# monahand1023/imageclust

Measured on AMD Instinct MI355X. Metric: images/sec (embed+Ward), higher is better.
Workload: dtype bf16; 1 GPU; the metric's size (configs[2]'s N=100000) on 1 GPU: 100000 synthetic 224x224x3 images (structured, seed 20250217; 100000 on this rank), ResNet50-v1 bf16 batch=256 -> 2048-d pooled E -> Ward min=5 max=50 (merge loop on GPU0) -> cluster ids on host; n_images_total=100000, embed_dim=2048, weights=synthetic seed 1, device=AMD Radeon Graphics (gfx950:sramecc+:xnack-)

## Files before the change

imageclust_amd/_lib.py:

```python
import ctypes as C
import os

import numpy as np

_HERE = os.path.dirname(os.path.abspath(__file__))
SO_PATH = os.environ.get("ICL_SO_PATH") or os.path.join(_HERE, "libimageclust_hip.so")

ICL_OK = 0
ICL_ERR_ARG, ICL_ERR_CONSTRAINT, ICL_ERR_HIP, ICL_ERR_NOMODEL, ICL_ERR_IO, ICL_ERR_UNSUPPORTED, ICL_ERR_OVERSIZE, ICL_ERR_NOMEM = range(1, 9)
HEAD_POOLED, HEAD_DENSE0 = 2048, 1000
PREC_FP32, PREC_BF16, PREC_BF16X3 = 0, 1, 2
UPDATE_EXACT, UPDATE_LW = 0, 1
SYNTH_NOISE, SYNTH_STRUCTURED = 0, 1
TILES_AUTO, TILES_LOCAL, TILES_DISTRIBUTED = 0, 1, 2
MERGE_GPU0, MERGE_SHARDED = 0, 1
CONV_P8_OFF, CONV_P8_AUTO, CONV_P8_ALL = 0, 1, 2
CONV_SPLIT = 16
ROWS_SINGLE, ROWS_EXACT_BATCH, ROWS_LW_BOUND, ROWS_LW_FAST = 0, 1, 2, 3
FILE_FAIL_NEXT_LEADER = 0x100
MANY_MID_AUTO, MANY_MID_OFF, MANY_MID_ON = 0, 1, 2
ENTROPY_HOST, ENTROPY_GPU = 0, 1
K_CONV, K_DIST_EXACT, K_DIST_MFMA, K_ROWMIN, K_UPDATE, K_EMBED_OTHER, K_CONV64 = range(7)
K_NAMES = ["conv_igemm_kernel<*,128>", "ward_dist_exact_kernel", "dist_mfma_kernel", "row_argmin_*_kernel",
           "ward_update_exact_kernel", "embed_other", "conv_igemm_kernel<*,64>"]
# ... 20 lines not shown
    ("icl_synthetic_blob_bytes", _i64, []),
    ("icl_synthetic_blob", _int, [C.c_uint64, _vp, _i64]),
    ("icl_embed_u8", _int, [_vp, _vp, _i64, _int, _int, _vp]),
    ("icl_embed_u8_dev", _int, [_vp, _vp, _i64, _int, _int, _vp]),
    ("icl_embed_file", _int, [_vp, C.c_char_p, _int, _vp]),
    ("icl_set_file_options", _int, [_vp, _int, _int, _int]),
    ("icl_file_batch_stats", _int, [_vp, _pi64, _pi64]),
    ("icl_preprocess_u8", _int, [_vp, _vp]),
    ("icl_preprocess_file", _int, [C.c_char_p, _vp]),
    ("icl_resize_u8", _int, [_vp, _i32, _i32, _vp, _i32, _i32]),
    ("icl_decode_image_file", _int, [C.c_char_p, _vp, _i64, _pi32, _pi32]),
    ("icl_load_image_224", _int, [C.c_char_p, _vp]),
    ("icl_load_images_224_dev", _int, [_vp, _vp, _i64, _i32, _vp, _vp]),
    ("icl_embed_files", _int, [_vp, _vp, _i64, _int, _int, _i32, _vp, _vp]),
    ("icl_embed_files_dev", _int, [_vp, _vp, _i64, _int, _int, _i32, _vp, _vp]),
    ("icl_last_ingest_stats", _int, [_vp, _pi64, _pi64, _pi64, _pd]),
    ("icl_set_ingest_options", _int, [_vp, _int]),
    ("icl_last_entropy_stats", _int, [_vp, _pi64, _pi64, _pi64, _pi64]),
    ("icl_jpeg_coefs_files", _int, [_vp, _vp, _i64, _int, _vp, _i64, _vp, _vp]),
    ("icl_jpeg_coefs_file_host", _int, [C.c_char_p, _int, _vp, _i64, _pi64, _vp]),
    ("icl_decode_image_mem", _int, [_vp, _i64, _vp, _i64, _pi32, _pi32]),
    ("icl_load_image_224_mem", _int, [_vp, _i64, _vp]),
    ("icl_preprocess_mem", _int, [_vp, _i64, _vp]),
    ("icl_embed_image_mem", _int, [_vp, _vp, _i64, _int, _vp]),
    ("icl_load_images_224_mem_dev", _int, [_vp, _vp, _vp, _i64, _i32, _vp, _vp]),
    ("icl_embed_images_mem", _int, [_vp, _vp, _vp, _i64, _int, _int, _i32, _vp, _vp]),
    ("icl_embed_images_mem_dev", _int, [_vp, _vp, _vp, _i64, _int, _int, _i32, _vp, _vp]),
    ("icl_cluster_requests_mem", _int, [_vp, _i32] + [_vp] * 8 + [_int, _int, _i32] + [_vp] * 8),
    ("icl_jpeg_coefs_mem", _int, [_vp, _vp, _vp, _i64, _int, _vp, _i64, _vp, _vp]),
    ("icl_set_batch", _int, [_vp, _int]),
    ("icl_set_conv_options", _int, [_vp, _int]),
    ("icl_conv_stats", _int, [_vp, _vp, _vp]),
    ("icl_conv_split_launches", _int, [_vp, _vp]),
    ("icl_conv2d_fused", _int, [_vp, _int, _vp, _int, _int, _int, _vp, _int, _int, _int, _int, _vp, _vp, _vp, _int, _vp]),
    ("icl_conv2d_dual", _int, [_vp, _int, _vp, _int, _int, _int, _vp, _vp, _int, _int, _vp, _int, _int, _vp, _vp, _int, _vp]),
    ("icl_embed_taps", _int, [_vp, _int, _vp, _int, _int, _vp]),
    ("icl_stem_pool", _int, [_vp, _int, _vp, _int, _vp]),
    ("icl_bottleneck56", _int, [_vp, _vp, _int, _int, _int, _int] + [_vp] * 13),
    ("icl_calc_optimal_clusters", _int, [_i64, _i64, _i64, _pi64]),
    ("icl_ward_distance_matrix", _int, [_vp, _vp, _vp, _i64, _i32, _vp, _i64]),
    ("icl_ward_distance_matrix_dev", _int, [_vp, _vp, _vp, _i64, _i32, _vp, _i64]),
    ("icl_merge_centroid", _int, [_vp, _vp, _i64, _vp, _i64, _i32, _vp]),
    ("icl_update_distance_matrix", _int, [_vp, _vp, _i64, _i64, _vp, _vp, _i32, _i64, _i64, _vp, _i64]),
    ("icl_find_closest", _int, [_vp, _vp, _i64, _i64, _pi64, _pi64]),
    ("icl_find_closest_dev", _int, [_vp, _vp, _i64, _i64, _pi64, _pi64]),
    ("icl_group_create", _int, [_pi32, _i32, C.POINTER(_vp)]),
    ("icl_group_destroy", None, [_vp]),
    ("icl_group_size", _i32, [_vp]),
    ("icl_group_ctx", _vp, [_vp, _i32]),
    ("icl_group_last_error", C.c_char_p, [_vp]),
    ("icl_group_load_onnx", _int, [_vp, C.c_char_p]),
    ("icl_group_load_blob", _int, [_vp, _vp, _i64]),
    ("icl_group_load_synthetic", _int, [_vp, C.c_uint64]),
    ("icl_group_embed_u8", _int, [_vp, _vp, _i64, _int, _int, _vp]),
    ("icl_group_cluster", _int, [_vp, _vp, _i64, _i32, _i32, _i32, _int, _vp, _vp, _pi32]),
    ("icl_set_ward_options", _int, [_vp, _int]),
    ("icl_embed_cluster_dev", _int, [_vp, _vp, _i64, _int, _i32, _i32, _int, _int, _vp, _vp, _vp, _pi32]),
    ("icl_group_embed_cluster", _int, [_vp, _vp, _i64, _int, _i32, _i32, _int, _vp, _vp, _vp, _pi32]),
    ("icl_ward_rows_partition", _int, [_i64, _i32, _i32, _pi64, _pi64]),
    ("icl_ward_span", _int, [_i64, _i64, _pi64, _pi64]),
    ("icl_ward_distance_rows_dev", _int, [_vp, _vp, _i64, _i32, _i64, _i64, _vp]),
    ("icl_ward_rows_hold_bounds", _int, [_vp, _i64, _int]),
    ("icl_ward_prepare", _int, [_vp, _i64, _i32]),
    ("icl_ward_unpack_spans_dev", _int, [_vp, _i32, _pi64, _pi64, C.POINTER(_vp)]),
    ("icl_group_set_options", _int, [_vp, _int, _int]),
    ("icl_cluster_prefilled_dev", _int, [_vp, _vp, _i64, _i32, _i32, _i32, _int, _i64, _i64, _vp, _vp, _pi32]),
# ... 249 lines not shown

        t = E if isinstance(E, torch.Tensor) else torch.from_numpy(np.ascontiguousarray(E, dtype=np.float32))
        t = t.to("cuda:%d" % self.device, dtype=torch.float32).contiguous()
        n, d = t.shape
        a, b, u = C.c_int64(0), C.c_int64(0), C.c_int64(0)
        g, v = C.c_double(0), C.c_double(0)
        check(self.h, self.L.icl_distance_bounds_check_dev(self.h, C.c_void_p(t.data_ptr()), n, d, kind, C.byref(a), C.byref(b), C.byref(u), C.byref(g), C.byref(v)))
        pairs = n * (n - 1) / 2
        return {"below": a.value, "above": b.value, "unflagged": u.value, "mean_gap": g.value / pairs, "mean_val": v.value / pairs}

    def load_synthetic(self, seed=1):
        check(self.h, self.L.icl_model_load_synthetic(self.h, seed))

    def load_blob(self, blob):
        buf = np.frombuffer(blob, np.uint8)
        check(self.h, self.L.icl_model_load_blob(self.h, buf.ctypes.data, buf.nbytes))

    def load_onnx(self, path):
        check(self.h, self.L.icl_model_load_onnx(self.h, os.fsencode(path)))

    def set_batch(self, b):
        check(self.h, self.L.icl_set_batch(self.h, b))

    def conv_stats(self):
        a, b = C.c_int64(0), C.c_int64(0)
        check(self.h, self.L.icl_conv_stats(self.h, C.byref(a), C.byref(b)))
        return a.value, b.value

    def conv_split_launches(self):
        a = C.c_int64(0)
        check(self.h, self.L.icl_conv_split_launches(self.h, C.byref(a)))
        return a.value

    def set_conv_options(self, p8_mode=1):
        check(self.h, self.L.icl_set_conv_options(self.h, p8_mode))

    def embed_u8(self, imgs, head=HEAD_POOLED, prec=PREC_FP32):
        imgs = np.ascontiguousarray(imgs, np.uint8).reshape(-1, IMG_BYTES)
        n = imgs.shape[0]
        out = np.empty((n, head), np.float32)
        check(self.h, self.L.icl_embed_u8(self.h, imgs.ctypes.data, n, head, prec, out.ctypes.data))
        return out

    def embed_u8_dev(self, d_imgs, n, d_out, head=HEAD_POOLED, prec=PREC_BF16):
        check(self.h, self.L.icl_embed_u8_dev(self.h, _vp(d_imgs), n, head, prec, _vp(d_out)))

    def embed_file(self, path, head=HEAD_DENSE0):
        out = np.empty(head, np.float32)
        check(self.h, self.L.icl_embed_file(self.h, os.fsencode(path), head, out.ctypes.data))
        return out

    def _files_call(self, fn, paths, *args):
        enc = [os.fsencode(p) for p in paths]
        arr = (C.c_char_p * max(1, len(enc)))(*enc)
        status = np.zeros(len(enc), np.int32)
        rc = fn(self.h, arr, len(enc), *args, status.ctypes.data)
        failed = np.flatnonzero(status)
        if rc != ICL_OK and not (failed.size and status[failed[0]] == rc):
            check(self.h, rc)
        return status

    def embed_image_mem(self, data, head=HEAD_DENSE0):
        p, n, keep = _byte_view(data)
        out = np.empty(head, np.float32)
        check(self.h, self.L.icl_embed_image_mem(self.h, _vp(p), n, head, out.ctypes.data))
        del keep
# ... 569 lines not shown
```

imageclust_amd/csrc/conv_wr.h:

```cpp
#pragma once
#include "mfma_tile.h"
#include "resnet_fused.h"

template <int NP>
__device__ __forceinline__ void wr_dma_chunk(const i32x4_t &srd, unsigned v0, unsigned v1, unsigned soff, unsigned lds0)
{
    unsigned keep;
    if constexpr (NP == 2)
        asm volatile("s_mov_b32 %0, m0\n\ts_mov_b32 m0, %5\n\ts_nop 4\n\tbuffer_load_dwordx4 %1, %3, %4 offen lds\n\t"
                     "s_mov_b32 m0, %6\n\ts_nop 0\n\tbuffer_load_dwordx4 %2, %3, %4 offen lds\n\ts_mov_b32 m0, %0"
                     : "=&s"(keep)
                     : "v"(v0), "v"(v1), "s"(srd), "s"(soff), "s"(lds0), "s"(lds0 + 4096u)
                     : "memory");
    else
        asm volatile("s_mov_b32 %0, m0\n\ts_mov_b32 m0, %4\n\ts_nop 4\n\tbuffer_load_dwordx4 %1, %2, %3 offen lds\n\ts_mov_b32 m0, %0"
                     : "=&s"(keep)
                     : "v"(v0), "s"(srd), "s"(soff), "s"(lds0)
                     : "memory");
}
template <int KC, int PT>
__device__ __forceinline__ void wr_dma(const i32x4_t &srd, unsigned v0, unsigned v1, unsigned lds0)
{
    static_assert(PT == 64 || PT == 32, "64- or 32-pixel tiles");
#pragma unroll
    for (int c = 0; c < KC; ++c) wr_dma_chunk<PT / 32>(srd, v0, v1, 128u * c, lds0 + (unsigned)(PT * 128) * c);
}

struct wr_args {
    const uint16_t *X;
    const uint16_t *W;
    const uint16_t *R;
    uint16_t *Y;
    const float *scale, *shift;
    int M, N, relu;
    int nslices, nworkers;
};

template <int K, int NS, int MT, bool RES>
__global__ __launch_bounds__(256, (K == 256 && MT == 2) ? 3 : 2) void conv_wr_kernel(const wr_args p)
{
    typedef unsigned u32x2_t __attribute__((ext_vector_type(2)));
    typedef unsigned u32x4_t __attribute__((ext_vector_type(4)));
    constexpr int KC = K / 64, KF = K / 32;
    constexpr int CW = NS / 4, NT = CW / 16;
    constexpr int PT = 16 * MT;
    constexpr int ABYTES = KC * PT * 128;
    static_assert(NT % 2 == 0 && NT * KF * 4 <= 128 && (MT == 4 || MT == 2), "pairs of accumulator tiles for the lane swap; <= 128 VGPRs of weights");
    __shared__ __attribute__((aligned(1024))) unsigned char smem[2 * ABYTES];
    const int tid = threadIdx.x, lane = tid & 63;
    const int wid = __builtin_amdgcn_readfirstlane(tid >> 6);
    const int l15 = lane & 15, q = lane >> 4;
    const int xcd = (int)blockIdx.x & 7, rr = (int)blockIdx.x >> 3;
    const int slice = rr % p.nslices, worker = (rr / p.nslices) * 8 + xcd;
    const int n0 = slice * NS + wid * CW;
    const int ntiles = (p.M + PT - 1) / PT;
    if (worker >= ntiles) return;

    u32x4_t wreg[NT][KF];
#pragma unroll
    for (int nt = 0; nt < NT; ++nt)
#pragma unroll
        for (int kf = 0; kf < KF; ++kf) wreg[nt][kf] = *reinterpret_cast<const u32x4_t *>(p.W + (size_t)(n0 + 16 * nt + l15) * K + 32 * kf + 8 * q);
    asm volatile("s_waitcnt vmcnt(0)" ::: "memory");
#pragma unroll
    for (int nt = 0; nt < NT; ++nt)
#pragma unroll
        for (int kf = 0; kf < KF; ++kf) asm volatile("" : "+v"(wreg[nt][kf]));
    const int cbl = (q & 1) * 16 + (q >> 1) * 8;
    float sc[NT / 2][8], sh[NT / 2][8];
#pragma unroll
    for (int i = 0; i < NT / 2; ++i) {
        const int c = n0 + i * 32 + cbl;
        const float4 a0 = *reinterpret_cast<const float4 *>(p.scale + c), a1 = *reinterpret_cast<const float4 *>(p.scale + c + 4);
        const float4 b0 = *reinterpret_cast<const float4 *>(p.shift + c), b1 = *reinterpret_cast<const float4 *>(p.shift + c + 4);
        sc[i][0] = a0.x; sc[i][1] = a0.y; sc[i][2] = a0.z; sc[i][3] = a0.w; sc[i][4] = a1.x; sc[i][5] = a1.y; sc[i][6] = a1.z; sc[i][7] = a1.w;
        sh[i][0] = b0.x; sh[i][1] = b0.y; sh[i][2] = b0.z; sh[i][3] = b0.w; sh[i][4] = b1.x; sh[i][5] = b1.y; sh[i][6] = b1.z; sh[i][7] = b1.w;
    }
    const i32x4_t xsrd = bn56_srd(p.X, (unsigned)((size_t)p.M * K * 2));
    const unsigned lds0 = __builtin_amdgcn_readfirstlane(lds_addr_of(smem) + wid * 1024);
    int drow[2];
    unsigned dsw[2];
#pragma unroll
    for (int j = 0; j < 2; ++j) {
        drow[j] = (j * 4 + wid) * 8 + (lane >> 3);
        dsw[j] = (unsigned)(((lane & 7) ^ ((drow[j] >> 1) & 7)) << 4);
    }
    auto stage = [&](int tile, int buf) {
        unsigned v[2];
#pragma unroll
        for (int j = 0; j < 2; ++j) {
            const int m = tile * PT + drow[j];
            v[j] = (tile < ntiles && m < p.M) ? (unsigned)m * (unsigned)(K * 2) + dsw[j] : BN56_OOB;
        }
        wr_dma<KC, PT>(xsrd, v[0], v[1], lds0 + buf * ABYTES);
    };
    const int fsw = (l15 >> 1) & 7;
    unsigned xoff[2];
#pragma unroll
    for (int s = 0; s < 2; ++s) xoff[s] = (unsigned)(l15 * 128 + ((((4 * s + q) ^ fsw) & 7) << 4));

    typedef uint16_t elem;
    const __amdgpu_buffer_rsrc_t rsrd = __builtin_amdgcn_make_buffer_rsrc((void *)(RES ? p.R : p.Y), 0, (int)((size_t)p.M * p.N * 2), 0x00020000);
    const __amdgpu_buffer_rsrc_t ysrd = __builtin_amdgcn_make_buffer_rsrc((void *)p.Y, 0, (int)((size_t)p.M * p.N * 2), 0x00020000);
    u32x4_t rv[MT][NT / 2];
    auto row_off = [&](int tile, int mt) -> unsigned {
        const int64_t m = (int64_t)tile * PT + mt * 16 + l15;
        return (tile < ntiles && m < p.M) ? (unsigned)((m * p.N + n0 + cbl) * 2) : BN56_OOB;
    };
    auto load_res = [&](int tile) {
        if (!RES) return;
#pragma unroll
        for (int mt = 0; mt < MT; ++mt) {
            const unsigned o = row_off(tile, mt);
#pragma unroll
            for (int i = 0; i < NT / 2; ++i) rv[mt][i] = __builtin_amdgcn_raw_buffer_load_b128(rsrd, (int)o, i * 64, 0);
        }
    };
    int tile = worker;
    stage(tile, 0);
    stage(tile + p.nworkers, 1);
    load_res(tile);
    asm volatile("s_waitcnt vmcnt(0)" ::: "memory");
    for (int it = 0; tile < ntiles; ++it, tile += p.nworkers) {
        const int buf = it & 1;
        __builtin_amdgcn_s_barrier();
        __builtin_amdgcn_sched_barrier(0);
        f32x4 acc[MT][NT];
// ... 26 lines not shown
        }
#pragma unroll
        for (int mt = 0; mt < MT; ++mt) {
            const unsigned o = row_off(tile, mt);
#pragma unroll
            for (int i = 0; i < NT / 2; ++i) {
                const f32x4 ta = acc[mt][2 * i], tb = acc[mt][2 * i + 1];
                float v[8];
#pragma unroll
                for (int j = 0; j < 4; ++j) {
                    const u32x2_t r = __builtin_amdgcn_permlane16_swap(__float_as_uint(ta[j]), __float_as_uint(tb[j]), false, false);
                    v[j] = __uint_as_float(r[0]);
                    v[4 + j] = __uint_as_float(r[1]);
                }
                const elem *re = reinterpret_cast<const elem *>(&rv[mt][i]);
                u32x4_t ov;
                elem *oe = reinterpret_cast<elem *>(&ov);
#pragma unroll
                for (int e = 0; e < 8; ++e) {
                    float y = v[e] * sc[i][e] + sh[i][e];
                    if (RES) y += BF16::to_f(re[e]);
                    if (p.relu) y = fmaxf(y, 0.0f);
                    oe[e] = BF16::from_f(y);
                }
                __builtin_amdgcn_raw_buffer_store_b128(ov, ysrd, (int)o, i * 64, 0);
            }
        }
        stage(tile + 2 * p.nworkers, buf);
        load_res(tile + p.nworkers);
    }
    asm volatile("s_waitcnt vmcnt(0)" ::: "memory");
}

static bool conv_wr_shape(const conv_args &a, int *ns, int *pt)
{
    static const int pt256 = [] {
        const char *e = getenv("ICL_WR_PT256");
        return e && atoi(e) == 32 ? 32 : 64;
    }();
    if (a.K == 128) { *ns = 256; *pt = 64; }
    else if (a.K == 256) { *ns = 128; *pt = pt256; }
    else if (a.K == 512) { *ns = 128; *pt = 32; }
    else return false;
    return a.Cout % *ns == 0;
}
static bool conv_wr_eligible(const conv_args &a, int mode)
{
    if (mode == 0 || a.X2 || a.KH != 1 || a.KW != 1 || a.stride != 1 || a.pad != 0 || a.Cin != a.K) return false;
    int ns, pt;
    if (!conv_wr_shape(a, &ns, &pt)) return false;
    if (a.K == 512 && a.Cout > 128 && a.Cout < 2048) return false;
    if ((size_t)a.M * a.K * 2 >= (1ull << 31) || (size_t)a.M * a.Cout * 2 >= (1ull << 31)) return false;
    return true;
}
template <int K, int NS, int MT>
static void launch_conv_wr_t(hipStream_t strm, const wr_args &w, dim3 grid, bool res)
{
    if (res) hipLaunchKernelGGL((conv_wr_kernel<K, NS, MT, true>), grid, dim3(256), 0, strm, w);
    else hipLaunchKernelGGL((conv_wr_kernel<K, NS, MT, false>), grid, dim3(256), 0, strm, w);
}
static void launch_conv_wr(icl_ctx *ctx, const conv_args &a)
{
    hipStream_t strm = ctx->cur_stream ? ctx->cur_stream : ctx->stream;
    wr_args w;
    w.X = (const uint16_t *)a.X; w.W = (const uint16_t *)a.Wt; w.R = (const uint16_t *)a.R; w.Y = (uint16_t *)a.Y;
    w.scale = a.scale; w.shift = a.shift; w.M = (int)a.M; w.N = a.Cout; w.relu = a.relu;
    int ns = 0, pt = 0;
    (void)conv_wr_shape(a, &ns, &pt);
    w.nslices = a.Cout / ns;
    const int ntiles = (int)icl_ceil_div(a.M, pt);
    const int per_cu = (a.K == 256 && pt == 32) ? 3 : 2;
    const int slots = per_cu * ctx->prop.multiProcessorCount;
    int nworkers = std::max(8, (slots / w.nslices) & ~7);
    nworkers = std::min(nworkers, (int)icl_ceil_div(ntiles, 8) * 8);
    w.nworkers = nworkers;
    const dim3 grid((unsigned)(w.nslices * nworkers));
    if (a.K == 128) launch_conv_wr_t<128, 256, 4>(strm, w, grid, a.R != nullptr);
    else if (a.K == 256 && pt == 64) launch_conv_wr_t<256, 128, 4>(strm, w, grid, a.R != nullptr);
    else if (a.K == 256) launch_conv_wr_t<256, 128, 2>(strm, w, grid, a.R != nullptr);
    else launch_conv_wr_t<512, 128, 2>(strm, w, grid, a.R != nullptr);
}
```

imageclust_amd/csrc/icl_common.h:

```cpp
#pragma once
#include <hip/hip_runtime.h>

#include <condition_variable>
#include <cstdarg>
#include <cstdint>
#include <cstdio>
#include <functional>
#include <mutex>
#include <string>
#include <vector>

#include "../../include/icl_model_format.h"
#include "../../include/imageclust.h"

#define ICL_MAXF 3.40282346638528859811704183484516925e+38f

struct icl_prof_slot {
    double ms = 0, flops = 0, bytes = 0;
    int64_t launches = 0;
};

struct icl_pending_event {
    hipEvent_t a, b;
    int kclass;
// ... 39 lines not shown
};

struct icl_sk_slot {
    hipStream_t stream = nullptr;
    void *part = nullptr;
    int *flag = nullptr;
    int cap = 0, epoch = 0;
};

struct icl_ward_report {
    std::vector<int32_t> merges;
    std::vector<float> merge_vals;
    int64_t bound_viol = 0;
    int32_t mode[2] = {0, 0};
    int64_t layout[3] = {0, 0, 0};
    int64_t stats[4] = {0, 0, 0, 0};
    double dist_ms = 0, merge_ms = 0;
};

struct icl_ctx {
    int device = 0;
    hipStream_t stream = nullptr;
    hipStream_t stream2 = nullptr;
    hipStream_t stream3 = nullptr;
    hipEvent_t ev_s3 = nullptr;
    std::function<int(int64_t, int64_t, hipEvent_t)> embed_hook;
    hipStream_t cur_stream = nullptr;
    hipEvent_t ev_fork = nullptr, ev_join = nullptr;
    std::mutex mu;
    std::string err;
    hipDeviceProp_t prop;
    int batch = 256;
    int64_t conv_launches[2] = {0, 0};
    int conv_wr = 1;
    int conv_sk = 0;
    int conv_sk_min_k = 2048;
    int64_t conv_sk_launches = 0;
    icl_sk_slot sk[8];
    int conv_p8 = 1;
    int ward_dist = 0;
    int prof_mask = 0;
    icl_prof_slot prof[ICL_K_NCLASS];
    std::vector<icl_pending_event> pending;
    std::vector<hipEvent_t> event_pool;
    double last_embed_ms = 0;
    icl_ward_report last;
    int64_t ward_wide_fail_n = 0;
    icl_model *model = nullptr;
    icl_ward_ws *ward = nullptr;
    icl_ward_shard *shard = nullptr;
    int shard_rank = 0;
    int64_t *ward_rowoff = nullptr;
    int64_t ward_rowoff_n = 0;
    void *file_batcher = nullptr;
    icl_many_ws *many = nullptr;
    int many_mid = 0;
    int64_t many_stats[4] = {0, 0, 0, 0};
    icl_ingest_ws *ingest = nullptr;
    int64_t ingest_stats[3] = {0, 0, 0};
    double ingest_decode_s = 0;
    int entropy_mode = 0;
    int64_t entropy_stats[4] = {0, 0, 0, 0};
    icl_requests_ws *requests = nullptr;
    double requests_ms[3] = {0, 0, 0};
    std::vector<const void *> lds_optin;
};

// ... 142 lines not shown
```

imageclust_amd/csrc/icl_core.hip:

```cpp
#include "icl_common.h"

#include <cstring>

static thread_local std::string g_tls_err;

int icl_fail(icl_ctx *ctx, int code, const char *fmt, ...)
{
    char buf[1024];
    va_list ap;
    va_start(ap, fmt);
    vsnprintf(buf, sizeof buf, fmt, ap);
    va_end(ap);
    if (ctx) ctx->err = buf;
    g_tls_err = buf;
    return code;
}

extern "C" const char *icl_version(void) { return "imageclust_hip 0.1 (gfx950)"; }

extern "C" const char *icl_last_error(icl_ctx *ctx) { return ctx ? ctx->err.c_str() : g_tls_err.c_str(); }

extern "C" int icl_create(int device, icl_ctx **out)
{
    if (!out) return icl_fail(nullptr, ICL_ERR_ARG, "icl_create: out is NULL");
// ... 3 lines not shown
    if (e != hipSuccess || ndev <= 0)
        return icl_fail(nullptr, ICL_ERR_HIP, "icl_create: no HIP device available (%s); this library has no CPU fallback",
                        e != hipSuccess ? hipGetErrorString(e) : "device count 0");
    if (device < 0 || device >= ndev) return icl_fail(nullptr, ICL_ERR_ARG, "icl_create: device %d out of range [0,%d)", device, ndev);
    icl_ctx *c = new icl_ctx();
    c->device = device;
    icl_device_guard g(device);
    if (!g.ok) {
        delete c;
        return icl_fail(nullptr, ICL_ERR_HIP, "icl_create: hipSetDevice(%d) failed", device);
    }
    e = hipGetDeviceProperties(&c->prop, device);
    if (e != hipSuccess) {
        delete c;
        return icl_fail(nullptr, ICL_ERR_HIP, "hipGetDeviceProperties: %s", hipGetErrorString(e));
    }
    if (strncmp(c->prop.gcnArchName, "gfx950", 6) != 0) {
        std::string arch = c->prop.gcnArchName;
        delete c;
        return icl_fail(nullptr, ICL_ERR_HIP, "icl_create: device %d is %s; this library is built for gfx950 only", device, arch.c_str());
    }
    e = hipStreamCreateWithFlags(&c->stream, hipStreamNonBlocking);
    if (e != hipSuccess) {
        delete c;
        return icl_fail(nullptr, ICL_ERR_HIP, "hipStreamCreate: %s", hipGetErrorString(e));
    }
    if (hipStreamCreateWithFlags(&c->stream2, hipStreamNonBlocking) != hipSuccess ||
        hipEventCreateWithFlags(&c->ev_fork, hipEventDisableTiming) != hipSuccess ||
        hipEventCreateWithFlags(&c->ev_join, hipEventDisableTiming) != hipSuccess) {
        (void)hipStreamDestroy(c->stream);
        delete c;
        return icl_fail(nullptr, ICL_ERR_HIP, "icl_create: side stream / events");
    }
    if (const char *ew = getenv("ICL_CONV_WR")) c->conv_wr = atoi(ew) != 0;
    if (const char *es = getenv("ICL_CONV_SK")) c->conv_sk = atoi(es) != 0;
    if (const char *ek = getenv("ICL_CONV_SK_MINK")) c->conv_sk_min_k = std::max(512, atoi(ek));
    if (const char *e8 = getenv("ICL_CONV_P8")) {
        const int v = atoi(e8);
        if (v >= ICL_CONV_P8_OFF && v <= ICL_CONV_P8_ALL) c->conv_p8 = v;
    }
    if (const char *ej = getenv("ICL_JPEG_ENTROPY")) c->entropy_mode = strcmp(ej, "gpu") == 0 ? ICL_ENTROPY_GPU : ICL_ENTROPY_HOST;
    if (const char *em = getenv("ICL_MANY_MID"))
        c->many_mid = strcmp(em, "on") == 0 ? ICL_MANY_MID_ON : strcmp(em, "off") == 0 ? ICL_MANY_MID_OFF : ICL_MANY_MID_AUTO;
    *out = c;
    return ICL_OK;
}

extern "C" void icl_destroy(icl_ctx *ctx)
{
    if (!ctx) return;
    icl_device_guard g(ctx->device);
    (void)hipStreamSynchronize(ctx->stream);
    icl_model_free(ctx);
    icl_ward_free(ctx);
    icl_file_batcher_free(ctx);
    icl_ingest_free(ctx);
    icl_many_free(ctx);
    icl_requests_free(ctx);
    for (auto &p : ctx->pending) {
        (void)hipEventDestroy(p.a);
        (void)hipEventDestroy(p.b);
    }
    for (auto ev : ctx->event_pool) (void)hipEventDestroy(ev);
    for (auto &s : ctx->sk) {
        if (s.part) (void)hipFree(s.part);
        if (s.flag) (void)hipFree(s.flag);
    }
// ... 68 lines not shown
        ICL_HIP(ctx, hipMemcpyAsync(dst, src, (size_t)bytes, hipMemcpyDeviceToHost, ctx->stream));
        ICL_HIP(ctx, hipStreamSynchronize(ctx->stream));
    }
    return ICL_OK;
}

extern "C" int icl_set_batch(icl_ctx *ctx, int batch)
{
    if (!ctx || batch < 1 || batch > 1024) return icl_fail(ctx, ICL_ERR_ARG, "icl_set_batch: batch must be in [1,1024]");
    std::lock_guard<std::mutex> lk(ctx->mu);
    ctx->batch = batch;
    return ICL_OK;
}

extern "C" int icl_set_conv_options(icl_ctx *ctx, int p8_mode)
{
    const int mode = p8_mode & ~ICL_CONV_SPLIT;
    if (!ctx || p8_mode < 0 || mode < ICL_CONV_P8_OFF || mode > ICL_CONV_P8_ALL)
        return icl_fail(ctx, ICL_ERR_ARG, "icl_set_conv_options: p8_mode must be 0, 1 or 2 (| ICL_CONV_SPLIT)");
    std::lock_guard<std::mutex> lk(ctx->mu);
    ctx->conv_p8 = mode;
    ctx->conv_sk = (p8_mode & ICL_CONV_SPLIT) ? 1 : 0;
    return ICL_OK;
}

extern "C" int icl_conv_split_launches(icl_ctx *ctx, int64_t *launches)
{
    if (!ctx || !launches) return icl_fail(ctx, ICL_ERR_ARG, "icl_conv_split_launches: NULL argument");
    std::lock_guard<std::mutex> lk(ctx->mu);
    *launches = ctx->conv_sk_launches;
    return ICL_OK;
}

extern "C" int icl_conv_stats(icl_ctx *ctx, int64_t *p8_launches, int64_t *other_launches)
{
    if (!ctx) return icl_fail(ctx, ICL_ERR_ARG, "icl_conv_stats: ctx is NULL");
    std::lock_guard<std::mutex> lk(ctx->mu);
    if (p8_launches) *p8_launches = ctx->conv_launches[0];
    if (other_launches) *other_launches = ctx->conv_launches[1];
    return ICL_OK;
}

static hipEvent_t take_event(icl_ctx *c)
{
    if (!c->event_pool.empty()) {
        hipEvent_t e = c->event_pool.back();
        c->event_pool.pop_back();
        return e;
    }
    hipEvent_t e = nullptr;
    (void)hipEventCreate(&e);
    return e;
}

icl_prof_scope::icl_prof_scope(icl_ctx *ctx, int kclass, double flops, double bytes) : c(ctx), k(kclass)
{
    if (!((c->prof_mask >> k) & 1)) return;
    c->prof[k].flops += flops;
    c->prof[k].bytes += bytes;
    c->prof[k].launches += 1;
    a = take_event(c);
    b = take_event(c);
    (void)hipEventRecord(a, c->stream);
}

icl_prof_scope::~icl_prof_scope()
// ... 96 lines not shown
```

imageclust_amd/csrc/resnet.hip:

```cpp
#include "icl_common.h"
#include "mfma_tile.h"
#include "resnet_model.h"

#include <algorithm>
#include <cmath>
#include <cstring>
#include <new>
#include <thread>
#include <type_traits>
#include <vector>

struct conv_args {
    const void *X;
    const void *Wt;
    void *Y;
    const void *R;
    const float *scale;
    const float *shift;
    const void *zero;
    int B, H, W, Cin, Ho, Wo, Cout, KH, KW, stride, pad, relu;
    int64_t M;
    int K;
    int gx, gy;
    const void *X2;
// ... 659 lines not shown
        for (int off = 32; off > 0; off >>= 1) s += __shfl_down(s, off, 64);
        if (lane == 0) y[b * nout + o] = s + bias[o];
    }
}

template <typename T, int BN, bool DUAL, int NST, bool EARLY = false>
static void launch_conv_variant(icl_ctx *ctx, conv_args &a, int nst_lds)
{
    icl_lds_optin(ctx, (const void *)conv_igemm_kernel<T, BN, DUAL, NST, EARLY>, (int)conv_lds_bytes<BN>(NST));
    a.gy = a.Cout / BN;
    hipLaunchKernelGGL((conv_igemm_kernel<T, BN, DUAL, NST, EARLY>), dim3((unsigned)(a.gx * a.gy)), dim3(256), conv_lds_bytes<BN>(nst_lds), ctx->cur_stream ? ctx->cur_stream : ctx->stream,
                       a);
}

template <typename T>
static int launch_conv_t(icl_ctx *ctx, conv_args a)
{
    constexpr bool X3 = is_x3<T>::value;
    const double flops = 2.0 * (double)a.M * a.Cout * a.K;
    if (X3) {
        a.Cin *= 2;
        a.Cin2 *= 2;
        a.K *= 2;
    }
    a.gx = (int)icl_ceil_div(a.M, CV_BM);
    const int nk = a.K / T::BK;
    static const int mode = [] {
        const char *e = getenv("ICL_CONV_MODE");
        return e ? atoi(e) : 1;
    }();
    const bool early = mode != 0;
    const bool wide = a.Cout % 128 == 0;
    icl_prof_scope ps(ctx, wide ? ICL_K_CONV : ICL_K_CONV64, flops, 0.0);
    if (std::is_same<T, BF16>::value && ctx->conv_wr && conv_wr_eligible(a, ctx->conv_p8)) {
        launch_conv_wr(ctx, a);
        ++ctx->conv_launches[0];
        ICL_HIP(ctx, hipGetLastError());
        return ICL_OK;
    }
    if ((std::is_same<T, BF16>::value || X3) && conv_p8_eligible(a, ctx->conv_p8)) {
        launch_conv_p8<X3>(ctx, a);
        ++ctx->conv_launches[0];
        ICL_HIP(ctx, hipGetLastError());
        return ICL_OK;
    }
    ++ctx->conv_launches[1];
    if (mode == 1 && !a.X2 && a.KH == 3 && a.KW == 3 && a.stride == 1 && a.pad == 1 && a.Ho == a.H && a.Wo == a.W && a.Cin >= 128) {
        const int npw = conv3x3_halo_npw(a.W);
        if (npw) {
            if (wide) launch_conv3x3_halo<T, 128>(ctx, a, npw);
            else launch_conv3x3_halo<T, 64>(ctx, a, npw);
            ICL_HIP(ctx, hipGetLastError());
            return ICL_OK;
        }
    }
    const int nst = nk > 1 ? 2 : 1;
    if (a.X2) {
        if (early) launch_conv_variant<T, 128, true, 2, true>(ctx, a, 2);
        else launch_conv_variant<T, 128, true, 2>(ctx, a, 2);
    } else if (wide) {
        if (early) launch_conv_variant<T, 128, false, 2, true>(ctx, a, nst);
        else launch_conv_variant<T, 128, false, 2>(ctx, a, nst);
    } else {
        if (early) launch_conv_variant<T, 64, false, 2, true>(ctx, a, nst);
        else launch_conv_variant<T, 64, false, 2>(ctx, a, nst);
    }
    ICL_HIP(ctx, hipGetLastError());
// ... 566 lines not shown
```

include/imageclust.h:

```cpp
#ifndef IMAGECLUST_H
#define IMAGECLUST_H
#include <stdint.h>

#ifdef __cplusplus
extern "C" {
#endif

typedef struct icl_ctx icl_ctx;

enum {
    ICL_OK = 0,
    ICL_ERR_ARG = 1,
    ICL_ERR_CONSTRAINT = 2,
    ICL_ERR_HIP = 3,
    ICL_ERR_NOMODEL = 4,
    ICL_ERR_IO = 5,
    ICL_ERR_UNSUPPORTED = 6,
    ICL_ERR_OVERSIZE = 7,
    ICL_ERR_NOMEM = 8
};

enum { ICL_HEAD_POOLED = 2048,
       ICL_HEAD_DENSE0 = 1000   };
enum { ICL_PREC_FP32 = 0,
// ... 21 lines not shown
int64_t icl_synthetic_blob_bytes(void);
int icl_synthetic_blob(uint64_t seed, void *blob, int64_t bytes);

int icl_embed_u8(icl_ctx *ctx, const uint8_t *hwc_rgb, int64_t n, int head, int prec, float *out);
int icl_embed_u8_dev(icl_ctx *ctx, const uint8_t *d_hwc_rgb, int64_t n, int head, int prec, float *d_out);
int icl_embed_file(icl_ctx *ctx, const char *path, int head, float *out);
enum { ICL_FILE_FAIL_NEXT_LEADER = 0x100 };
int icl_set_file_options(icl_ctx *ctx, int prec, int window_us, int max_batch);
int icl_file_batch_stats(icl_ctx *ctx, int64_t *batches, int64_t *images);
int icl_decode_image_file(const char *path, uint8_t *rgb, int64_t cap_bytes, int32_t *w, int32_t *h);
int icl_load_image_224(const char *path, uint8_t *out);
int icl_preprocess_u8(const uint8_t *hwc_rgb, float *nchw);
int icl_preprocess_file(const char *path, float *nchw);
int icl_resize_u8(const uint8_t *src_rgb, int32_t sw, int32_t sh, uint8_t *dst_rgb, int32_t dw, int32_t dh);
int icl_load_images_224_dev(icl_ctx *ctx, const char *const *paths, int64_t n, int32_t threads,
                            uint8_t *d_out , int32_t *status);
int icl_embed_files(icl_ctx *ctx, const char *const *paths, int64_t n, int head, int prec,
                    int32_t threads, float *out, int32_t *status);
int icl_embed_files_dev(icl_ctx *ctx, const char *const *paths, int64_t n, int head, int prec,
                        int32_t threads, float *d_out, int32_t *status);
int icl_last_ingest_stats(icl_ctx *ctx, int64_t *gpu_jpegs, int64_t *host_files, int64_t *upload_bytes,
                          double *host_decode_s);
enum { ICL_ENTROPY_HOST = 0, ICL_ENTROPY_GPU = 1 };
int icl_set_ingest_options(icl_ctx *ctx, int entropy_mode);
int icl_last_entropy_stats(icl_ctx *ctx, int64_t *gpu_entropy_jpegs, int64_t *host_entropy_jpegs, int64_t *redone_on_host,
                           int64_t *stream_bytes);
int icl_jpeg_coefs_files(icl_ctx *ctx, const char *const *paths, int64_t n, int entropy_mode, int16_t *coefs, int64_t cap,
                         int64_t *offsets , int32_t *state );
int icl_jpeg_coefs_file_host(const char *path, int sub_bits, int16_t *coefs, int64_t cap, int64_t *need, int32_t *info );
int icl_set_batch(icl_ctx *ctx, int batch);
enum { ICL_CONV_P8_OFF = 0, ICL_CONV_P8_AUTO = 1, ICL_CONV_P8_ALL = 2, ICL_CONV_SPLIT = 16 };
int icl_set_conv_options(icl_ctx *ctx, int p8_mode);
int icl_conv_split_launches(icl_ctx *ctx, int64_t *launches);
int icl_conv_stats(icl_ctx *ctx, int64_t *p8_launches, int64_t *other_launches);
int icl_conv2d_fused(icl_ctx *ctx, int prec, const float *x, int B, int H, int Cin, const float *w, int Cout, int k,
                     int stride, int pad, const float *scale, const float *shift, const float *residual, int relu,
                     float *y);

int icl_conv2d_dual(icl_ctx *ctx, int prec, const float *x, int B, int Ho, int Cin, const float *w1, const float *x2, int H2, int Cin2,
                    const float *w2, int stride2, int Cout, const float *scale, const float *shift, int relu, float *y);
int icl_embed_taps(icl_ctx *ctx, int prec, const uint8_t *hwc_rgb, int B, int tap, float *out);

int icl_stem_pool(icl_ctx *ctx, int prec, const uint8_t *hwc_rgb, int B, float *out);
int icl_bottleneck56(icl_ctx *ctx, const float *x, int B, int H, int W, int Cin, const float *w1, const float *sc1, const float *sh1,
                     const float *w2, const float *sc2, const float *sh2, const float *w3, const float *sc3, const float *sh3,
                     const float *wds, const float *scds, const float *shds, float *y);

typedef struct icl_group icl_group;
int icl_group_create(const int32_t *devices, int32_t ndev, icl_group **out);
void icl_group_destroy(icl_group *g);
int32_t icl_group_size(icl_group *g);
icl_ctx *icl_group_ctx(icl_group *g, int32_t i);
const char *icl_group_last_error(icl_group *g);
int icl_group_load_onnx(icl_group *g, const char *path);
int icl_group_load_blob(icl_group *g, const void *blob, int64_t bytes);
int icl_group_load_synthetic(icl_group *g, uint64_t seed);
int icl_group_embed_u8(icl_group *g, const uint8_t *hwc_rgb, int64_t n, int head, int prec, float *out);
int icl_group_cluster(icl_group *g, const float *E, int64_t n, int32_t d, int32_t min_size, int32_t max_size, int update,
                      int32_t *cluster_id, int32_t *member_rank, int32_t *n_clusters);
int icl_group_embed_cluster(icl_group *g, const uint8_t *hwc_rgb, int64_t n, int prec, int32_t min_size, int32_t max_size, int update,
                            float *E_out, int32_t *cluster_id, int32_t *member_rank, int32_t *n_clusters);

enum { ICL_TILES_AUTO = 0, ICL_TILES_LOCAL = 1, ICL_TILES_DISTRIBUTED = 2 };
enum { ICL_MERGE_GPU0 = 0, ICL_MERGE_SHARDED = 1 };
int icl_group_set_options(icl_group *g, int tiles_mode, int merge_mode);

// ... 103 lines not shown
```

scratch/isa_compare.py:

```python
#!/usr/bin/env python3
import re
import sys


def kernels(path):
    lines = open(path).read().split("\n")
    out = {}
    label = {ln.split(";")[0].strip(): i for i, ln in enumerate(lines) if ln[:1] not in (" ", "\t", "")}
    for i, ln in enumerate(lines):
        m = re.match(r"\s*\.amdhsa_kernel\s+(\S+)", ln)
        if not m:
            continue
        name = m.group(1)
        j = i
        while not lines[j].strip().startswith(".end_amdhsa_kernel"):
            j += 1
        desc = "\n".join(x.strip() for x in lines[i:j + 1])
        a = label[name + ":"]
        b = a
        while not lines[b].startswith(".Lfunc_end"):
            b += 1
        out[name] = (re.sub(r"\.LBB\d+_", ".LBB_", "\n".join(lines[a:b])), desc)
    return out


def main():
    pa, pb, rest = sys.argv[1], sys.argv[2], sys.argv[3:]
    A, B = kernels(pa), kernels(pb)
    bad = 0
    print("%s: %d kernels, %s: %d kernels, same names: %s" % (pa, len(A), pb, len(B), sorted(A) == sorted(B)))
    for name in sorted(set(A) | set(B)):
        if name not in A or name not in B:
            verdict = "only in " + (pa if name in A else pb)
        else:
            verdict = "identical" if A[name] == B[name] else "differs (%s)" % ("code" if A[name][0] != B[name][0] else "descriptor")
        bad += verdict != "identical"
        print("  %-9s %s" % (verdict, name))
    for p in rest:
        n = len(kernels(p))
        bad += n != 0
        print("%s: %d kernels (host-only unit: expected 0)" % (p, n))
    print("ALL IDENTICAL" if not bad else "%d DIFFERENCES" % bad)
    return 1 if bad else 0


if __name__ == "__main__":
    sys.exit(main())
```

Measured before the change: 70950 images/sec.

## Extend warp-resident 1x1 conv kernel to strided and dual-input downsample layers

Generalizes the conv_wr 1x1 conv kernel so it also handles strided 1x1 convolutions (K=256/512) and the fused dual-input downsample path (Cin=128 plus a strided Cin2=256 input). The address computation maps output pixels to strided input pixels, and a second buffer descriptor feeds the second operand into the same LDS tile. The default conv_wr bitmask enables stride-1, strided and dual sets, while strided K=512 stays off. The intent is to move these layers off the generic implicit-GEMM path onto the faster DMA-to-LDS kernel, at the cost of per-row integer division and new kernel instantiations that may carry higher register pressure. It also adds a launch counter and profiling scripts.

```diff
diff --git a/imageclust_amd/_lib.py b/imageclust_amd/_lib.py
--- a/imageclust_amd/_lib.py
+++ b/imageclust_amd/_lib.py
@@ -76,6 +76,7 @@
     ("icl_set_conv_options", _int, [_vp, _int]),
     ("icl_conv_stats", _int, [_vp, _vp, _vp]),
     ("icl_conv_split_launches", _int, [_vp, _vp]),
+    ("icl_conv_wr_launches", _int, [_vp, _vp]),
     ("icl_conv2d_fused", _int, [_vp, _int, _vp, _int, _int, _int, _vp, _int, _int, _int, _int, _vp, _vp, _vp, _int, _vp]),
     ("icl_conv2d_dual", _int, [_vp, _int, _vp, _int, _int, _int, _vp, _vp, _int, _int, _vp, _int, _int, _vp, _vp, _int, _vp]),
     ("icl_embed_taps", _int, [_vp, _int, _vp, _int, _int, _vp]),
@@ -391,6 +392,11 @@
         check(self.h, self.L.icl_conv_split_launches(self.h, C.byref(a)))
         return a.value
 
+    def conv_wr_launches(self):
+        a = C.c_int64(0)
+        check(self.h, self.L.icl_conv_wr_launches(self.h, C.byref(a)))
+        return a.value
+
     def set_conv_options(self, p8_mode=1):
         check(self.h, self.L.icl_set_conv_options(self.h, p8_mode))
 
diff --git a/imageclust_amd/csrc/conv_wr.h b/imageclust_amd/csrc/conv_wr.h
--- a/imageclust_amd/csrc/conv_wr.h
+++ b/imageclust_amd/csrc/conv_wr.h
@@ -26,6 +26,15 @@
     for (int c = 0; c < KC; ++c) wr_dma_chunk<PT / 32>(srd, v0, v1, 128u * c, lds0 + (unsigned)(PT * 128) * c);
 }
 
+template <int KC, int KC1, int PT>
+__device__ __forceinline__ void wr_dma2(const i32x4_t &srd, const i32x4_t &srd2, const unsigned (&v)[2], const unsigned (&v2)[2], unsigned lds0)
+{
+#pragma unroll
+    for (int c = 0; c < KC1; ++c) wr_dma_chunk<PT / 32>(srd, v[0], v[1], 128u * c, lds0 + (unsigned)(PT * 128) * c);
+#pragma unroll
+    for (int c = KC1; c < KC; ++c) wr_dma_chunk<PT / 32>(srd2, v2[0], v2[1], 128u * (c - KC1), lds0 + (unsigned)(PT * 128) * c);
+}
+
 struct wr_args {
     const uint16_t *X;
     const uint16_t *W;
@@ -35,10 +44,19 @@
     int M, N, relu;
     int nslices, nworkers;
 };
-
-template <int K, int NS, int MT, bool RES>
-__global__ __launch_bounds__(256, (K == 256 && MT == 2) ? 3 : 2) void conv_wr_kernel(const wr_args p)
-{
+struct wr_args_s : wr_args {
+    const uint16_t *X2;
+    int IH, IW, Ho, Wo, stride;
+    unsigned xbytes, x2bytes;
+};
+
+template <int AF>
+using wr_args_of = typename std::conditional<AF == 0, wr_args, wr_args_s>::type;
+
+template <int K, int NS, int MT, bool RES, int AF = 0>
+__global__ __launch_bounds__(256, ((K == 256 && MT == 2) || K == 384) ? 3 : 2) void conv_wr_kernel(const wr_args_of<AF> p)
+{
+    static_assert(AF == 0 || (!RES && (AF == 1 || (AF == 2 && K > 128))), "stride 1, strided or dual; the strided and dual layers have no residual");
     typedef unsigned u32x2_t __attribute__((ext_vector_type(2)));
     typedef unsigned u32x4_t __attribute__((ext_vector_type(4)));
     constexpr int KC = K / 64, KF = K / 32;
@@ -76,7 +94,15 @@
         sc[i][0] = a0.x; sc[i][1] = a0.y; sc[i][2] = a0.z; sc[i][3] = a0.w; sc[i][4] = a1.x; sc[i][5] = a1.y; sc[i][6] = a1.z; sc[i][7] = a1.w;
         sh[i][0] = b0.x; sh[i][1] = b0.y; sh[i][2] = b0.z; sh[i][3] = b0.w; sh[i][4] = b1.x; sh[i][5] = b1.y; sh[i][6] = b1.z; sh[i][7] = b1.w;
     }
-    const i32x4_t xsrd = bn56_srd(p.X, (unsigned)((size_t)p.M * K * 2));
+    constexpr int K1 = AF == 2 ? 128 : K;
+    const i32x4_t xsrd = bn56_srd(p.X, [&] {
+        if constexpr (AF == 0) return (unsigned)((size_t)p.M * K * 2);
+        else return p.xbytes;
+    }());
+    const i32x4_t x2srd = [&] {
+        if constexpr (AF == 2) return bn56_srd(p.X2, p.x2bytes);
+        else return xsrd;
+    }();
     const unsigned lds0 = __builtin_amdgcn_readfirstlane(lds_addr_of(smem) + wid * 1024);
     int drow[2];
     unsigned dsw[2];
@@ -86,13 +112,33 @@
         dsw[j] = (unsigned)(((lane & 7) ^ ((drow[j] >> 1) & 7)) << 4);
     }
     auto stage = [&](int tile, int buf) {
-        unsigned v[2];
-#pragma unroll
-        for (int j = 0; j < 2; ++j) {
-            const int m = tile * PT + drow[j];
-            v[j] = (tile < ntiles && m < p.M) ? (unsigned)m * (unsigned)(K * 2) + dsw[j] : BN56_OOB;
-        }
-        wr_dma<KC, PT>(xsrd, v[0], v[1], lds0 + buf * ABYTES);
+        if constexpr (AF == 0) {
+            unsigned v[2];
+#pragma unroll
+            for (int j = 0; j < 2; ++j) {
+                const int m = tile * PT + drow[j];
+                v[j] = (tile < ntiles && m < p.M) ? (unsigned)m * (unsigned)(K * 2) + dsw[j] : BN56_OOB;
+            }
+            wr_dma<KC, PT>(xsrd, v[0], v[1], lds0 + buf * ABYTES);
+        } else {
+            unsigned v[2] = {BN56_OOB, BN56_OOB}, v2[2] = {BN56_OOB, BN56_OOB};
+#pragma unroll
+            for (int j = 0; j < PT / 32; ++j) {
+                const int m = tile * PT + drow[j];
+                if (tile < ntiles && m < p.M) {
+                    const unsigned tq = (unsigned)m / (unsigned)p.Wo, ox = (unsigned)m - tq * (unsigned)p.Wo;
+                    const unsigned b = tq / (unsigned)p.Ho, oy = tq - b * (unsigned)p.Ho;
+                    const unsigned pix = (b * (unsigned)p.IH + oy * (unsigned)p.stride) * (unsigned)p.IW + ox * (unsigned)p.stride;
+                    if constexpr (AF == 1) v[j] = pix * (unsigned)(K * 2) + dsw[j];
+                    else {
+                        v[j] = (unsigned)m * (unsigned)(K1 * 2) + dsw[j];
+                        v2[j] = pix * (unsigned)((K - K1) * 2) + dsw[j];
+                    }
+                }
+            }
+            if constexpr (AF == 1) wr_dma<KC, PT>(xsrd, v[0], v[1], lds0 + buf * ABYTES);
+            else wr_dma2<KC, K1 / 64, PT>(xsrd, x2srd, v, v2, lds0 + buf * ABYTES);
+        }
     };
     const int fsw = (l15 >> 1) & 7;
     unsigned xoff[2];
@@ -185,25 +231,42 @@
     asm volatile("s_waitcnt vmcnt(0)" ::: "memory");
 }
 
+enum { WR_SET_STRIDE1 = 1, WR_SET_STRIDED = 2, WR_SET_DUAL = 4, WR_SET_STRIDED_512 = 8 };
 static bool conv_wr_shape(const conv_args &a, int *ns, int *pt)
 {
     static const int pt256 = [] {
         const char *e = getenv("ICL_WR_PT256");
         return e && atoi(e) == 32 ? 32 : 64;
     }();
-    if (a.K == 128) { *ns = 256; *pt = 64; }
-    else if (a.K == 256) { *ns = 128; *pt = pt256; }
+    if (a.X2) {
+        if (a.Cin != 128 || a.Cin2 != 256) return false;
+        *ns = 128; *pt = 32;
+    }
+    else if (a.K == 128) { *ns = 256; *pt = 64; }
+    else if (a.K == 256) { *ns = 128; *pt = a.stride == 1 ? pt256 : 64; }
     else if (a.K == 512) { *ns = 128; *pt = 32; }
     else return false;
     return a.Cout % *ns == 0;
 }
-static bool conv_wr_eligible(const conv_args &a, int mode)
-{
-    if (mode == 0 || a.X2 || a.KH != 1 || a.KW != 1 || a.stride != 1 || a.pad != 0 || a.Cin != a.K) return false;
+static bool conv_wr_eligible(const conv_args &a, int mode, int sets)
+{
+    if (mode == 0 || a.KH != 1 || a.KW != 1 || a.pad != 0 || a.stride < 1 || a.K != a.Cin + (a.X2 ? a.Cin2 : 0)) return false;
     int ns, pt;
     if (!conv_wr_shape(a, &ns, &pt)) return false;
+    if (a.M < 1 || (size_t)a.M * a.Cout * 2 >= (1ull << 31)) return false;
+    if ((size_t)a.B * a.H * a.W * a.Cin * 2 >= (1ull << 31)) return false;
+    if (a.X2) {
+        if (!(sets & WR_SET_DUAL) || mode != 1 || a.R || a.stride != 1 || a.stride2 < 1) return false;
+        if ((int64_t)(a.Ho - 1) * a.stride2 >= a.H2 || (int64_t)(a.Wo - 1) * a.stride2 >= a.W2) return false;
+        return (size_t)a.B * a.H2 * a.W2 * a.Cin2 * 2 < (1ull << 31);
+    }
+    if (a.stride != 1) {
+        if (!(sets & WR_SET_STRIDED) || mode != 1 || a.R || (a.K != 256 && a.K != 512)) return false;
+        if (a.K == 512 && !(sets & WR_SET_STRIDED_512)) return false;
+        return (int64_t)(a.Ho - 1) * a.stride < a.H && (int64_t)(a.Wo - 1) * a.stride < a.W;
+    }
+    if (!(sets & WR_SET_STRIDE1)) return false;
     if (a.K == 512 && a.Cout > 128 && a.Cout < 2048) return false;
-    if ((size_t)a.M * a.K * 2 >= (1ull << 31) || (size_t)a.M * a.Cout * 2 >= (1ull << 31)) return false;
     return true;
 }
 template <int K, int NS, int MT>
@@ -215,19 +278,30 @@
 static void launch_conv_wr(icl_ctx *ctx, const conv_args &a)
 {
     hipStream_t strm = ctx->cur_stream ? ctx->cur_stream : ctx->stream;
-    wr_args w;
+    wr_args_s w;
     w.X = (const uint16_t *)a.X; w.W = (const uint16_t *)a.Wt; w.R = (const uint16_t *)a.R; w.Y = (uint16_t *)a.Y;
     w.scale = a.scale; w.shift = a.shift; w.M = (int)a.M; w.N = a.Cout; w.relu = a.relu;
     int ns = 0, pt = 0;
     (void)conv_wr_shape(a, &ns, &pt);
     w.nslices = a.Cout / ns;
     const int ntiles = (int)icl_ceil_div(a.M, pt);
-    const int per_cu = (a.K == 256 && pt == 32) ? 3 : 2;
+    const int per_cu = (a.K == 384 || (a.K == 256 && pt == 32)) ? 3 : 2;
     const int slots = per_cu * ctx->prop.multiProcessorCount;
     int nworkers = std::max(8, (slots / w.nslices) & ~7);
     nworkers = std::min(nworkers, (int)icl_ceil_div(ntiles, 8) * 8);
     w.nworkers = nworkers;
     const dim3 grid((unsigned)(w.nslices * nworkers));
+    ++ctx->conv_wr_launches;
+    if (a.X2 || a.stride != 1) {
+        w.X2 = (const uint16_t *)a.X2;
+        w.IH = a.X2 ? a.H2 : a.H; w.IW = a.X2 ? a.W2 : a.W; w.Ho = a.Ho; w.Wo = a.Wo; w.stride = a.X2 ? a.stride2 : a.stride;
+        w.xbytes = (unsigned)((size_t)a.B * a.H * a.W * a.Cin * 2);
+        w.x2bytes = a.X2 ? (unsigned)((size_t)a.B * a.H2 * a.W2 * a.Cin2 * 2) : 0u;
+        if (a.X2) hipLaunchKernelGGL((conv_wr_kernel<384, 128, 2, false, 2>), grid, dim3(256), 0, strm, w);
+        else if (a.K == 256) hipLaunchKernelGGL((conv_wr_kernel<256, 128, 4, false, 1>), grid, dim3(256), 0, strm, w);
+        else hipLaunchKernelGGL((conv_wr_kernel<512, 128, 2, false, 1>), grid, dim3(256), 0, strm, w);
+        return;
+    }
     if (a.K == 128) launch_conv_wr_t<128, 256, 4>(strm, w, grid, a.R != nullptr);
     else if (a.K == 256 && pt == 64) launch_conv_wr_t<256, 128, 4>(strm, w, grid, a.R != nullptr);
     else if (a.K == 256) launch_conv_wr_t<256, 128, 2>(strm, w, grid, a.R != nullptr);
diff --git a/imageclust_amd/csrc/icl_common.h b/imageclust_amd/csrc/icl_common.h
--- a/imageclust_amd/csrc/icl_common.h
+++ b/imageclust_amd/csrc/icl_common.h
@@ -95,7 +95,8 @@
     hipDeviceProp_t prop;
     int batch = 256;
     int64_t conv_launches[2] = {0, 0};
-    int conv_wr = 1;
+    int conv_wr = 7;
+    int64_t conv_wr_launches = 0;
     int conv_sk = 0;
     int conv_sk_min_k = 2048;
     int64_t conv_sk_launches = 0;
diff --git a/imageclust_amd/csrc/icl_core.hip b/imageclust_amd/csrc/icl_core.hip
--- a/imageclust_amd/csrc/icl_core.hip
+++ b/imageclust_amd/csrc/icl_core.hip
@@ -59,7 +59,7 @@
         delete c;
         return icl_fail(nullptr, ICL_ERR_HIP, "icl_create: side stream / events");
     }
-    if (const char *ew = getenv("ICL_CONV_WR")) c->conv_wr = atoi(ew) != 0;
+    if (const char *ew = getenv("ICL_CONV_WR")) c->conv_wr = atoi(ew) & 15;
     if (const char *es = getenv("ICL_CONV_SK")) c->conv_sk = atoi(es) != 0;
     if (const char *ek = getenv("ICL_CONV_SK_MINK")) c->conv_sk_min_k = std::max(512, atoi(ek));
     if (const char *e8 = getenv("ICL_CONV_P8")) {
@@ -194,6 +194,14 @@
     return ICL_OK;
 }
 
+extern "C" int icl_conv_wr_launches(icl_ctx *ctx, int64_t *launches)
+{
+    if (!ctx || !launches) return icl_fail(ctx, ICL_ERR_ARG, "icl_conv_wr_launches: NULL argument");
+    std::lock_guard<std::mutex> lk(ctx->mu);
+    *launches = ctx->conv_wr_launches;
+    return ICL_OK;
+}
+
 extern "C" int icl_conv_stats(icl_ctx *ctx, int64_t *p8_launches, int64_t *other_launches)
 {
     if (!ctx) return icl_fail(ctx, ICL_ERR_ARG, "icl_conv_stats: ctx is NULL");
diff --git a/imageclust_amd/csrc/resnet.hip b/imageclust_amd/csrc/resnet.hip
--- a/imageclust_amd/csrc/resnet.hip
+++ b/imageclust_amd/csrc/resnet.hip
@@ -715,7 +715,7 @@
     const bool early = mode != 0;
     const bool wide = a.Cout % 128 == 0;
     icl_prof_scope ps(ctx, wide ? ICL_K_CONV : ICL_K_CONV64, flops, 0.0);
-    if (std::is_same<T, BF16>::value && ctx->conv_wr && conv_wr_eligible(a, ctx->conv_p8)) {
+    if (std::is_same<T, BF16>::value && ctx->conv_wr && conv_wr_eligible(a, ctx->conv_p8, ctx->conv_wr)) {
         launch_conv_wr(ctx, a);
         ++ctx->conv_launches[0];
         ICL_HIP(ctx, hipGetLastError());
diff --git a/include/imageclust.h b/include/imageclust.h
--- a/include/imageclust.h
+++ b/include/imageclust.h
@@ -77,6 +77,7 @@
 enum { ICL_CONV_P8_OFF = 0, ICL_CONV_P8_AUTO = 1, ICL_CONV_P8_ALL = 2, ICL_CONV_SPLIT = 16 };
 int icl_set_conv_options(icl_ctx *ctx, int p8_mode);
 int icl_conv_split_launches(icl_ctx *ctx, int64_t *launches);
+int icl_conv_wr_launches(icl_ctx *ctx, int64_t *launches);
 int icl_conv_stats(icl_ctx *ctx, int64_t *p8_launches, int64_t *other_launches);
 int icl_conv2d_fused(icl_ctx *ctx, int prec, const float *x, int B, int H, int Cin, const float *w, int Cout, int k,
                      int stride, int pad, const float *scale, const float *shift, const float *residual, int relu,
diff --git a/scratch/isa_compare.py b/scratch/isa_compare.py
--- a/scratch/isa_compare.py
+++ b/scratch/isa_compare.py
@@ -20,13 +20,27 @@
         b = a
         while not lines[b].startswith(".Lfunc_end"):
             b += 1
-        out[name] = (re.sub(r"\.LBB\d+_", ".LBB_", "\n".join(lines[a:b])), desc)
+        body = "\n".join(x.split(";")[0].rstrip() for x in lines[a:b])
+        out[name] = (re.sub(r"\.LBB\d+_", ".LBB_", body).replace(name, "<kernel>"), desc.replace(name, "<kernel>"))
     return out
 
 
 def main():
-    pa, pb, rest = sys.argv[1], sys.argv[2], sys.argv[3:]
-    A, B = kernels(pa), kernels(pb)
+    argv, renames = sys.argv[1:], []
+    while argv and argv[0] == "--rename":
+        renames.append((argv[1], argv[2]))
+        argv = argv[3:]
+    pa, pb, rest = argv[0], argv[1], argv[2:]
+
+    def renamed(d):
+        out = {}
+        for name, v in d.items():
+            for pat, repl in renames:
+                name = re.sub(pat, repl, name)
+            out[name] = v
+        return out
+
+    A, B = renamed(kernels(pa)), renamed(kernels(pb))
     bad = 0
     print("%s: %d kernels, %s: %d kernels, same names: %s" % (pa, len(A), pb, len(B), sorted(A) == sorted(B)))
     for name in sorted(set(A) | set(B)):
diff --git a/scratch/layer_lanes.py b/scratch/layer_lanes.py
--- /dev/null
+++ b/scratch/layer_lanes.py
@@ -0,0 +1,79 @@
+#!/usr/bin/env python3
+import csv
+import sys
+
+NBLOCKS = [3, 4, 6, 3]
+CONV = ("conv_igemm", "conv3x3_halo", "conv_p8", "conv_wr")
+
+
+def layer_names():
+    out = []
+    for s in range(1, 4):
+        for bl in range(NBLOCKS[s]):
+            out += ["s%d.b%d.c%d" % (s + 1, bl, c) for c in (1, 2, 3)]
+    return out
+
+
+def family(name):
+    for f, short in (("conv_wr", "wr"), ("conv_p8", "p8"), ("halo", "halo"), ("conv_igemm", "igemm")):
+        if f in name:
+            return short
+    return "?"
+
+
+def read(path):
+    rows = list(csv.DictReader(open(path)))
+    col = next((c for c in ("Stream_Id", "Queue_Id") if c in rows[0] and len({r[c] for r in rows}) > 1), None)
+    lanes = {}
+    for r in rows:
+        lanes.setdefault(r[col] if col else "0", []).append((int(r["Start_Timestamp"]), int(r["End_Timestamp"]), r["Kernel_Name"]))
+    names = layer_names()
+    per_layer = {n: [] for n in names}
+    fam, spans, nb = {}, [], 0
+    for ev in lanes.values():
+        ev.sort()
+        stems = [i for i, e in enumerate(ev) if "stem" in e[2][:40]]
+        for a, b in zip(stems[1:], stems[2:] + [len(ev)]):
+            batch = ev[a:b]
+            convs = [e for e in batch if any(k in e[2] for k in CONV)]
+            if len(convs) != len(names) or not any("avgpool" in e[2] for e in batch):
+                continue
+            nb += 1
+            last = max(i for i, e in enumerate(batch) if "avgpool" in e[2])
+            spans.append((batch[last][1] - batch[0][0]) / 1e3)
+            for (s, e, n), name in zip(convs, names):
+                per_layer[name].append((e - s) / 1e3)
+                fam[name] = family(n)
+    return per_layer, fam, spans, nb, len(lanes), col
+
+
+def stats(v):
+    m = sum(v) / len(v)
+    return m, min(v), (sum((x - m) ** 2 for x in v) / len(v)) ** 0.5
+
+
+def main():
+    args = sys.argv[1:]
+    only = None
+    if args and args[0] == "--layers":
+        only, args = args[1].split(","), args[2:]
+    traces = [(a.split("=", 1)[0], read(a.split("=", 1)[1])) for a in args]
+    for name, (_, _, spans, nb, nl, col) in traces:
+        print("%-14s %d lanes (by %s), %d batches, mean batch span %.1f us" % (name, nl, col or "one queue", nb, sum(spans) / max(len(spans), 1)))
+    print("%-9s" % "layer" + "".join("  %-32s" % ("%s: mean / min / sd us" % n) for n, _ in traces))
+    for layer in layer_names():
+        if only and layer not in only:
+            continue
+        line = "%-9s" % layer
+        for _, (pl, fam, _, _, _, _) in traces:
+            m, lo, sd = stats(pl[layer])
+            line += "  %7.1f / %7.1f / %5.1f %-6s" % (m, lo, sd, fam[layer])
+        print(line)
+    line = "%-9s" % "conv sum"
+    for _, (pl, _, _, _, _, _) in traces:
+        line += "  %7.1f %-25s" % (sum(stats(v)[0] for v in pl.values()), "(stages 2-4)")
+    print(line)
+
+
+if __name__ == "__main__":
+    main()
```

Result: no change. 71440 images/sec, median of 6 (+0.7%).
